# ImIntheMiddle/VATL4Pose-WACV2024

Hardware: AMD Instinct MI355X
Metric: frames/sec pose-infer+uncertainty, 256x192 17-kp (higher is better)
Workload: dtype f32; 1 GPU; SimpleBaseline-R50 256x192 inference + decode + local-peak + THC-L1, 1024-frame synthetic video per GPU; frames_per_gpu=1024, batch=1024, tracks=4, parallelism=frame-sharded x1

## Files before the change

### include/vatl_hip.h

```cpp
#ifndef VATL_HIP_H
#define VATL_HIP_H

#include <stdint.h>

#ifdef __cplusplus
extern "C" {
#endif

#define VATL_VERSION 100
#define VATL_EINVAL  (-1)
#define VATL_ELAUNCH (-2)

int         vatl_version(void);
const char* vatl_last_error(void);

int vatl_flop_meter_begin(void);
int vatl_flop_meter_end(double* direct_flops, double* winograd_flops, int64_t* direct_launches, int64_t* winograd_launches);
#define VATL_ROUTE_NAMES "igemm,igemm_bnbwd,igemm_dma,persistent_1x1,streamk,rows_1x1,bottleneck_chain,stem_pool,halo_3x3," \
                         "winograd,winograd_2h,winograd_bnbwd,winograd_persist,winograd_c32,wgrad,winograd_wgrad,winograd_wgrad_2h," \
                         "winograd_wgrad_table,winograd_f4,winograd_f4_bnbwd,gemm1x1_ring,winograd_deconv43,winograd_s2_43,stem_pool_w1d," \
                         "chain_proj,chain_step"
int vatl_flop_meter_routes(int64_t* counts, int n);


// ... 30 lines not shown
int64_t vatl_winograd_c32_weight_floats(void);
int vatl_pack_winograd_c32_weight(const float* w, float* u, void* stream);
int vatl_conv3x3_winograd_c32_supported(int N, int H, int W, int Cin, int Cout);
int vatl_conv3x3_winograd_c32_fwd(const float* x, const float* u, const float* scale, const float* bias, const float* residual, float* y, int N, int H, int W,
                                  int relu, void* stream);

int64_t vatl_winograd_f4_weight_floats(int Cout, int Cin);
int vatl_pack_winograd_f4_weight(const float* w, float* u, int Cout, int Cin, int data_gradient, void* stream);
int vatl_conv3x3_winograd_f4_supported(int N, int H, int W, int Cin, int Cout);
int vatl_conv3x3_winograd_f4_fwd(const float* x, const float* u, const float* scale, const float* bias, const float* residual, float* y, int N, int H, int W,
                                 int Cin, int Cout, int relu, void* stream);
int64_t vatl_winograd_f4_stats_row_blocks(int64_t N, int H, int W);
int vatl_conv3x3_winograd_f4_fwd_stats(const float* x, const float* u, float* y, double* stats, int64_t* row_blocks_used, int N, int H, int W, int Cin, int Cout,
                                       void* stream);
int vatl_conv3x3_winograd_f4_fwd_bnbwd(const float* x, const float* u, const float* residual, float* y, int N, int H, int W, int Cin, int Cout, const float* bn_z,
                                       const float* bn_mask_y, const float* bn_scale, const float* bn_bias, const float* bn_mean, const float* bn_invstd,
                                       double* stats, int64_t* row_blocks_used, void* stream);

int vatl_conv1x1_rows_supported(int K1, int K2, int N, int64_t M);
int vatl_conv1x1_rows_fwd(const float* a, const float* x2, const float* w, const float* scale, const float* bias, const float* residual, float* y,
                          int64_t M, int K1, int K2, int N, int relu, void* stream);

int vatl_bottleneck_chain_supported(int Cmid, int Cout, int Cnext, int64_t M);
int vatl_bottleneck_chain_fwd(const float* a, const float* w3, const float* scale3, const float* bias3, const float* skip, float* t,
                              const float* w1, const float* scale1, const float* bias1, float* y1, int64_t M, int Cmid, int Cout,
                              int Cnext, void* stream);

int vatl_chain_proj_supported(int Cmid, int Cout, int Cnext, int64_t M);
int vatl_chain_proj_fwd(const float* a, const float* x2, const float* w, const float* scale, const float* bias, float* t, const float* w1,
                        const float* scale1, const float* bias1, float* y1, int64_t M, int Cmid, int Cout, int Cnext, int relu, void* stream);
int vatl_chain_step_supported(int Cmid, int Cout, int Cnext, int64_t M);
int vatl_chain_step_fwd(const float* a, const float* w3, const float* scale3, const float* bias3, const float* skip, float* t, const float* w1,
                        const float* scale1, const float* bias1, float* y1, int64_t M, int Cmid, int Cout, int Cnext, void* stream);

int vatl_tune_set(int knob, int value);
int vatl_set_splitk_workspace(float* workspace, int64_t floats);
int vatl_set_splitk_workspace_thread(float* workspace, int64_t floats);
int64_t vatl_streamk_workspace_bytes(void);
int vatl_set_streamk_workspace_thread(void* workspace, int64_t bytes);
int vatl_conv_cout_pad(int Cout);
int vatl_conv2d_fwd(const float* x, const float* w, const float* scale, const float* bias, const float* residual,
                    float* y, int N, int H, int W, int Cin, int Cout, int CoutPad, int R, int S, int stride, int pad,
                    int relu, int out_nchw, void* stream);

int vatl_deconv4x4s2_fwd(const float* x, const float* w, const float* scale, const float* bias, float* y,
                         int N, int H, int W, int Cin, int Cout, int CoutPad, int relu, void* stream);

int vatl_maxpool3x3s2_fwd(const float* x, float* y, int N, int H, int W, int C, void* stream);
int vatl_gap_fwd(const float* x, float* y, int N, int HW, int C, void* stream);

int vatl_pixelshuffle2_fwd(const float* x, float* y, int N, int H, int W, int C, void* stream);
int vatl_se_scale_add_relu(const float* x, const float* gate, const float* residual, float* y, int N, int HW, int C, void* stream);
int vatl_fuse_upsample_add(const float* base, const float* z0, int shift0, const float* z1, int shift1, const float* z2, int shift2,
                           float* y, int N, int H, int W, int C, int relu, void* stream);
int vatl_upsample_nearest_bwd(const float* dy, const float* yact_or_null, float* dz, int N, int H, int W, int C, int shift, void* stream);
int vatl_gap_bwd(const float* dy, float* dx, int N, int HW, int C, void* stream);


int vatl_decode_argmax_affine(const float* hm, const float* bbox, float* coords, float* maxvals, int32_t* idx,
                              int N, int J, int H, int W, void* stream);
int vatl_decode_pose(const float* hm, const float* bbox, float* kpts, int32_t* idx, float* hp, double* pose_score,
                     int N, int J, int H, int W, void* stream);

int vatl_thc_pairs(const float* a, const float* b, int64_t stride_a, int64_t stride_b, float* out,
                   int P, int J, int HW, int norm, void* stream);
int vatl_thc_combine(const float* pair, const uint8_t* is_prev, const uint8_t* is_next, float* thc, int N, void* stream);
// ... 260 lines not shown
```

### vatl4pose-wacv2024_amd/alphapose/models/hip_engine.py

```python
from __future__ import annotations

import time
import weakref

import torch
import torch.nn as nn

import vatl_hip as vh

MAX_CHUNK = 1024



WINOGRAD = True
ROWS_GEMM = True
ROWS_GEMM_K = (128, 256)
WINO_C32 = True
WINO_F4 = True
DECONV_43 = True
S2_43 = True


class _Conv:
    __slots__ = ("w", "u", "u32", "u4", "us2", "wsrc", "wino", "c32", "f4", "s2", "scale", "bias", "cout", "r", "s", "stride", "pad")
# ... 83 lines not shown
        if WINOGRAD and dc.weight.shape[0] % 16 == 0 and self.cout % 4 == 0:
            self.u = vh.pack_winograd_deconv_weight(dc.weight.detach())
        self.w = vh.pack_deconv_weight(dc.weight.detach())
        self.scale, self.bias = vh.bn_fold(_d(bn.weight), _d(bn.bias), bn.running_mean, bn.running_var, bn.eps)

    def __call__(self, x, relu=True):
        if self.u is not None and not vh.latency_mode():
            if self.d43 and self.u43 is None and vh.deconv4x4s2_winograd43_supported(x.shape[0], x.shape[1], x.shape[2], x.shape[3], self.cout):
                self.u43 = vh.pack_winograd_deconv43_weight(self.wsrc)
            return vh.deconv4x4s2_winograd_fwd(x, self.u, self.scale, self.bias, self.cout, relu, u43=self.u43)
        return vh.deconv4x4s2_fwd(x, self.w, self.scale, self.bias, self.cout, relu)


def _d(p):
    return None if p is None else p.detach()


FUSE_PROJ = True


class _BottleneckPlan:
    def __init__(self, blk):
        self.c1 = _Conv(blk.conv1, blk.bn1)
        self.c2 = _DeformConv(blk) if getattr(blk, "with_dcn", False) else _Conv(blk.conv2, blk.bn2)
        self.c3 = _Conv(blk.conv3, blk.bn3)
        self.proj = _Conv(blk.downsample[0], blk.downsample[1]) if blk.downsample is not None else None
        self.dual = None
        if (FUSE_PROJ and self.proj is not None and type(self) is _BottleneckPlan and self.proj.r == 1 and self.c3.cout >= 128
                and blk.conv3.in_channels % 32 == 0 and blk.downsample[0].in_channels % 32 == 0):
            w, b = vh.pack_conv1x1_dual_weight(blk.conv3.weight.detach(), self.c3.scale, self.c3.bias, blk.downsample[0].weight.detach(),
                                               self.proj.scale, self.proj.bias)
            self.dual = (w, b, self.proj.stride)

    def __call__(self, x, out=None, y1=None, nxt=None):
        y = y1 if y1 is not None else self.c1(x, relu=True)
        y = self.c2(y, relu=True)
        return self.tail(y, x, out=out, nxt=nxt)

    def tail(self, y, x, out=None, nxt=None):
        if self.dual is not None:
            if (ROWS_GEMM and self.dual[2] == 1 and y.shape[-1] == 64 and x.shape[-1] == 64 and not vh.latency_mode()
                    and vh.conv1x1_rows_supported(64, 64, self.c3.cout, y.shape[0] * y.shape[1] * y.shape[2])):
                if nxt is not None and FUSE_CHAIN_PROJ and vh.chain_proj_supported(64, self.c3.cout, nxt[0].shape[0], y.shape[0] * y.shape[1] * y.shape[2]):
                    return vh.conv1x1_rows_fwd(y, self.dual[0], None, self.dual[1], self.c3.cout, True, x2=x, out=out, next_conv1=nxt)
                t = vh.conv1x1_rows_fwd(y, self.dual[0], None, self.dual[1], self.c3.cout, True, x2=x, out=out)
            else:
                t = vh.conv1x1_dual_fwd(y, x, self.dual[0], self.dual[1], self.c3.cout, self.dual[2], True, out=out)
        else:
            skip = x if self.proj is None else self.proj(x, relu=False)
            t = self.c3(y, relu=True, residual=skip, out=out)
        return t if nxt is None else (t, None)


FUSE_CHAIN = True
FUSE_CHAIN_PROJ = True
FUSE_CHAIN_STEP = True


def _conv1_of(nxt, cout):
    if (type(nxt) is _BottleneckPlan and (nxt.c1.r, nxt.c1.stride, nxt.c1.pad) == (1, 1, 0) and nxt.c1.scale is not None and nxt.c1.cout == cout
            and not vh.latency_mode()):
        return nxt.c1.w, nxt.c1.scale, nxt.c1.bias
    return None


def _run_blocks(blocks, x, out=None):
    y1 = None
    for k, b in enumerate(blocks):
        last = k == len(blocks) - 1
        o = out if last else None
        if type(b) is not _BottleneckPlan:
            x, y1 = b(x), None
            continue
        nxt = None if last else blocks[k + 1]
        m = x.shape[0] * x.shape[1] * x.shape[2]
        chain = (FUSE_CHAIN and b.proj is None and not vh.latency_mode() and b.c3.scale is not None
                 and vh.bottleneck_chain_supported(b.c3.w.shape[-1], b.c3.cout, 0, m))
        if not chain:
            c1 = _conv1_of(nxt, 64) if b.dual is not None and FUSE_CHAIN_PROJ else None
            x, y1 = b(x, out=o, y1=y1, nxt=c1) if c1 is not None else (b(x, out=o, y1=y1), None)
            continue
        y = b.c2(y1 if y1 is not None else b.c1(x, relu=True), relu=True)
        link, step = _conv1_of(nxt, 64), _conv1_of(nxt, 128) if FUSE_CHAIN_STEP else None
        if link is not None and vh.bottleneck_chain_supported(b.c3.w.shape[-1], b.c3.cout, 64, m):
            x, y1 = vh.bottleneck_chain_fwd(y, b.c3.w, b.c3.scale, b.c3.bias, x, *link, out=o)
        elif step is not None and vh.chain_step_supported(b.c3.w.shape[-1], b.c3.cout, 128, m):
            x, y1 = vh.bottleneck_chain_fwd(y, b.c3.w, b.c3.scale, b.c3.bias, x, out=o, next_stage_conv1=step)
        else:
            x, y1 = vh.bottleneck_chain_fwd(y, b.c3.w, b.c3.scale, b.c3.bias, x, out=o)[0], None
    return x


FUSE_STEM = True
STEM_W1D = True


def _stem_pool_weight(net):
    c = net.conv1
    ok = (FUSE_STEM and tuple(c.weight.shape) == (64, 3, 7, 7) and c.stride == (2, 2) and c.padding == (3, 3) and c.bias is None
          and isinstance(net.maxpool, nn.MaxPool2d) and net.maxpool.kernel_size in (3, (3, 3)) and net.maxpool.stride in (2, (2, 2))
          and net.maxpool.padding in (1, (1, 1)) and not net.maxpool.ceil_mode)
    return vh.pack_stem_pool_weight(c.weight.detach()) if ok else None


class _TrunkPlan:
    def __init__(self, net):
        self.stem = _Conv(net.conv1, net.bn1)
        self.stem_pw = _stem_pool_weight(net)
        self.stem_src, self.stem_u1d = net.conv1.weight.detach(), None
        self.blocks = [_BottleneckPlan(b) for stage in net.stages() for b in stage]

    def _stem(self, x_nchw):
        if self.stem_pw is not None and not vh.latency_mode() and vh.stem_pool_supported(x_nchw.shape[2], x_nchw.shape[3]):
            u1d = None
            if STEM_W1D and vh.stem_pool_w1d_supported(x_nchw.shape[2], x_nchw.shape[3]):
                if self.stem_u1d is None:
                    self.stem_u1d = vh.pack_stem_pool_w1d_weight(self.stem_src)
                u1d = self.stem_u1d
            return vh.stem_pool_fwd(x_nchw, self.stem_pw, self.stem.scale, self.stem.bias, u1d=u1d)
        x = vh.nchw_to_nhwc(x_nchw, 4)
# ... 398 lines not shown
```

### vatl4pose-wacv2024_amd/csrc/bottleneck_chain.hip

```cpp
#include "common.h"
#include "buffer.h"

namespace vatl {

struct ChainParams {
    const float* a;
    const float* w3;
    const float* scale3;
    const float* bias3;
    const float* res;
    float* t;
    const float* w1;
    const float* scale1;
    const float* bias1;
    float* out2;
    int M, N2, relu3;
    int m_tiles;
    unsigned a_bytes, t_bytes, o_bytes, w3_bytes, w1_bytes;
};

constexpr unsigned BOOB = 0xFFFFFFFFu;

constexpr int BT_LDT = 260;
constexpr int BT_AS = 32 * 64;
// ... 128 lines not shown
#pragma unroll
                    for (int w = 1; w < 4; ++w) {
                        const f32x4 q = *reinterpret_cast<const f32x4*>(&Ts[w * (32 * 68) + row * 68 + q4 * 4]);
#pragma unroll
                        for (int c = 0; c < 4; ++c) sum[c] += q[c];
                    }
                    f32x4 o;
#pragma unroll
                    for (int c = 0; c < 4; ++c) o[c] = fmaxf(sum[c] * s1[c] + b1[c], 0.f);
                    buf_store4(orr, ((unsigned)(mt * 32 + row) * 64u + (unsigned)q4 * 4u) * 4u, o);
                }
            }
        }
        if constexpr (SECOND) asm volatile("s_waitcnt vmcnt(10)" ::: "memory");
        else asm volatile("s_waitcnt vmcnt(8)" ::: "memory");
    }
}


struct FormParams {
    const float* a;
    const float* x2;
    const float* w3;
    const float* scale3;
    const float* bias3;
    const float* res;
    float* t;
    const float* w1;
    const float* scale1;
    const float* bias1;
    float* y;
    int m_tiles, relu3;
    unsigned a_bytes, t_bytes, y_bytes;
};

__device__ __forceinline__ unsigned uadd(unsigned s_part, unsigned v_part) {
#if defined(__HIP_DEVICE_COMPILE__)
    unsigned r;
    asm("v_add_u32 %0, %1, %2" : "=v"(r) : "s"(s_part), "v"(v_part));
    return r;
#else
    return s_part + v_part;
#endif
}

constexpr int CF_TS = 4 * 32 * 64;

template <bool PROJ>
__global__ __launch_bounds__(256, 2) void chain_form_kernel(FormParams p) {
    constexpr int K1 = PROJ ? 128 : 64, G1 = K1 / 8, AS = 32 * K1, N2 = PROJ ? 64 : 128;
    extern __shared__ __attribute__((aligned(16))) float smem[];
    float* As = smem;
    float* Ts = smem + 2 * AS;
    const int tid = threadIdx.x, lane = tid & 63, wave = __builtin_amdgcn_readfirstlane(tid >> 6);
    const int fr = lane & 31, h = lane >> 5;
    const int nblk = gridDim.x;

    const __amdgpu_buffer_rsrc_t ar = buf_rsrc(p.a, p.a_bytes);
    const __amdgpu_buffer_rsrc_t xr = buf_rsrc(PROJ ? p.x2 : p.a, PROJ ? p.a_bytes : 0u);
    const __amdgpu_buffer_rsrc_t w3r = buf_rsrc(p.w3, 256u * K1 * 4u);
    const __amdgpu_buffer_rsrc_t w1r = buf_rsrc(p.w1, (unsigned)N2 * 256u * 4u);
    const __amdgpu_buffer_rsrc_t tr = buf_rsrc(p.t, p.t_bytes);
    const __amdgpu_buffer_rsrc_t rr = buf_rsrc(p.res ? p.res : p.t, p.res ? p.t_bytes : 0u);
    const __amdgpu_buffer_rsrc_t yr = buf_rsrc(p.y, p.y_bytes);

    f32x4 w3f[2][G1];
#pragma unroll
    for (int nb = 0; nb < 2; ++nb)
#pragma unroll
        for (int g = 0; g < G1; ++g) w3f[nb][g] = buf_load4(w3r, (unsigned)(((wave * 64 + nb * 32 + fr) * K1 + 8 * g + 4 * h) * 4));
    float sc3[2], bi3[2];
#pragma unroll
    for (int nb = 0; nb < 2; ++nb) {
        const int n = wave * 64 + nb * 32 + fr;
        sc3[nb] = p.scale3 ? p.scale3[n] : 1.f;
        bi3[nb] = p.bias3 ? p.bias3[n] : 0.f;
    }
    const int l16 = lane & 15, j = lane >> 4;
    const int n1 = PROJ ? wave * 16 + l16 : wave * 32 + fr;
    f32x4 w1f[PROJ ? 16 : 32];
#pragma unroll
    for (int g = 0; g < (PROJ ? 16 : 32); ++g) w1f[g] = buf_load4(w1r, (unsigned)((n1 * 256 + (PROJ ? 16 * g + 4 * j : 8 * g + 4 * h)) * 4));
    const float sc1 = p.scale1 ? p.scale1[n1] : 1.f, bi1 = p.bias1 ? p.bias1[n1] : 0.f;
    const float lo3 = p.relu3 ? 0.f : -INFINITY;

    const int c4 = lane, r0 = wave;
    int ax[4], tq[4], tw[2], tx[PROJ ? 2 : 4];
#pragma unroll
    for (int k = 0; k < 4; ++k) {
        ax[k] = fr * K1 + (((2 * k + h) ^ (fr & 7)) << 2);
        tq[k] = 2 * AS + 4 * h * 64 + ((((fr >> 2) ^ (4 * h) ^ k) << 2) | (fr & 3));
    }
#pragma unroll
    for (int k = 0; k < 2; ++k) tw[k] = 2 * AS + (c4 >> 4) * 2048 + (((c4 & 15) ^ (r0 | 4 * k)) << 2);
#pragma unroll
// ... 27 lines not shown
            __builtin_amdgcn_raw_ptr_buffer_load_lds(rr, (lds_void*)(Ts + wave * 2048 + u * 256), 16,
                                                     uadd((unsigned)mt * (32u * 1024u) + (unsigned)u * 4096u + (unsigned)wave * 256u, vs[u & 1]), 0, 0, 0);
    };

    int mt = blockIdx.x, buf = 0;
    a_dma(0, mt);
    asm volatile("s_waitcnt vmcnt(0)" ::: "memory");
    for (; mt < p.m_tiles; mt += nblk, buf ^= 1) {
        lds_barrier();
        if constexpr (!PROJ) skip_dma(mt);
        a_dma(buf ^ 1, mt + nblk);
        __builtin_amdgcn_sched_barrier(0);
        const int abase = buf * AS, tqbase = wave * 2048;
#pragma unroll
        for (int nb = 0; nb < 2; ++nb) {
            f32x16 acc;
#pragma unroll
            for (int e = 0; e < 16; ++e) acc[e] = 0.f;
#pragma unroll
            for (int g = 0; g < G1; ++g) {
                const f32x4 af = *reinterpret_cast<const f32x4*>(smem + abase + ax[g & 3] + 32 * (g >> 2));
#pragma unroll
                for (int tt = 0; tt < 4; ++tt) acc = __builtin_amdgcn_mfma_f32_32x32x2f32(af[tt], w3f[nb][g][tt], acc, 0, 0, 0);
            }
            if (!PROJ && nb == 0) asm volatile("s_waitcnt vmcnt(2)" ::: "memory");
#pragma unroll
            for (int e = 0; e < 16; ++e) {
                float* q = smem + tqbase + tq[e & 3] + 64 * ((e & 3) + 8 * (e >> 2)) + 32 * nb;
                const float v = acc[e] * sc3[nb] + bi3[nb];
                *q = fmaxf(v + (PROJ ? 0.f : *q), lo3);
            }
        }
        lds_barrier();
#pragma unroll
        for (int u = 0; u < 8; ++u)
            buf_store4(tr, uadd((unsigned)mt * (32u * 1024u) + (unsigned)(r0 + 4 * u) * 1024u, (unsigned)c4 * 16u),
                       *reinterpret_cast<const f32x4*>(smem + r0 * 64 + tw[u & 1] + 256 * u));
        const unsigned ytile = (unsigned)mt * (32u * N2 * 4u) + (unsigned)wave * (PROJ ? 64u : 128u);
        if constexpr (PROJ) {
            f32x4 acc2[2] = {f32x4{0.f, 0.f, 0.f, 0.f}, f32x4{0.f, 0.f, 0.f, 0.f}};
#pragma unroll
            for (int q = 0; q < 16; ++q) {
                f32x4 tf[2];
#pragma unroll
                for (int rb = 0; rb < 2; ++rb) tf[rb] = *reinterpret_cast<const f32x4*>(smem + tx[q & 1] + 32 * ((q >> 1) & 1) + 2048 * (q >> 2) + 1024 * rb);
#pragma unroll
                for (int tt = 0; tt < 4; ++tt)
#pragma unroll
                    for (int rb = 0; rb < 2; ++rb) acc2[rb] = __builtin_amdgcn_mfma_f32_16x16x4f32(tf[rb][tt], w1f[q][tt], acc2[rb], 0, 0, 0);
            }
#pragma unroll
            for (int rb = 0; rb < 2; ++rb)
#pragma unroll
                for (int r = 0; r < 4; ++r) buf_store1(yr, uadd(ytile + (unsigned)(rb * 16 + r) * (N2 * 4u), vy), fmaxf(acc2[rb][r] * sc1 + bi1, 0.f));
            asm volatile("s_waitcnt vmcnt(16)" ::: "memory");
        } else {
            f32x16 acc2;
#pragma unroll
            for (int e = 0; e < 16; ++e) acc2[e] = 0.f;
#pragma unroll
            for (int g = 0; g < 32; ++g) {
                const f32x4 tf = *reinterpret_cast<const f32x4*>(smem + tx[g & 3] + 32 * ((g >> 2) & 1) + 2048 * (g >> 3));
#pragma unroll
                for (int tt = 0; tt < 4; ++tt) acc2 = __builtin_amdgcn_mfma_f32_32x32x2f32(tf[tt], w1f[g][tt], acc2, 0, 0, 0);
            }
#pragma unroll
            for (int e = 0; e < 16; ++e) buf_store1(yr, uadd(ytile + (unsigned)((e & 3) + 8 * (e >> 2)) * (N2 * 4u), vy), fmaxf(acc2[e] * sc1 + bi1 + 0.f, 0.f));
            asm volatile("s_waitcnt vmcnt(24)" ::: "memory");
        }
    }
}

}

using namespace vatl;

static bool chain_shape_ok(int Cmid, int Cout, int Cnext, int64_t M) {
    return Cmid == 64 && Cout == 256 && (Cnext == 64 || Cnext == 0) && M > 0 && (M + 32) * 256 < (1LL << 30);
}

extern "C" int vatl_bottleneck_chain_supported(int Cmid, int Cout, int Cnext, int64_t M) { return chain_shape_ok(Cmid, Cout, Cnext, M) ? 1 : 0; }

extern "C" int vatl_bottleneck_chain_fwd(const float* a, const float* w3, const float* scale3, const float* bias3, const float* skip, float* t, const float* w1,
                                         const float* scale1, const float* bias1, float* y1, int64_t M, int Cmid, int Cout, int Cnext, void* stream) {
    if (!a || !w3 || !t || (Cnext != 0) != (w1 != nullptr) || (w1 && !y1)) return fail(VATL_EINVAL, "bottleneck_chain_fwd: bad arguments");
    if (!chain_shape_ok(Cmid, Cout, Cnext, M)) return fail(VATL_EINVAL, "bottleneck_chain_fwd: serves 64 -> 256 (-> 64) channels and (M + 32) * 256 < 2^30 pixels x channels");
    ChainParams p{};
    p.a = a; p.w3 = w3; p.scale3 = scale3; p.bias3 = bias3; p.res = skip; p.t = t; p.w1 = w1; p.scale1 = scale1; p.bias1 = bias1; p.out2 = y1;
    p.M = (int)M; p.N2 = 64; p.relu3 = 1; p.m_tiles = (int)((M + 31) / 32);
    p.a_bytes = (unsigned)(M * 64 * 4); p.t_bytes = (unsigned)(M * 256 * 4); p.o_bytes = (unsigned)(M * 64 * 4); p.w3_bytes = 256 * 64 * 4; p.w1_bytes = 64 * 256 * 4;
    const int smem = BT_FLOATS * (int)sizeof(float);
    static std::atomic<unsigned> c0{0}, c1{0};
    const double padded = (double)p.m_tiles * 32.0;
    if (w1) {
        auto kern = bottleneck_chain_kernel<true>;
        if (int rc = ensure_dynamic_lds(reinterpret_cast<const void*>(kern), smem, c1, "bottleneck_chain")) return rc;
        const int grid = p.m_tiles < 512 ? p.m_tiles : 512;
        hipLaunchKernelGGL(kern, dim3(grid), dim3(256), smem, (hipStream_t)stream, p);
        meter_add(0, 2.0 * padded * 256.0 * 64.0 * 2.0);
        meter_route(kRouteChain);
    } else {
        auto kern = bottleneck_chain_kernel<false>;
        if (int rc = ensure_dynamic_lds(reinterpret_cast<const void*>(kern), smem, c0, "bottleneck_chain")) return rc;
        const int grid = p.m_tiles < 512 ? p.m_tiles : 512;
        hipLaunchKernelGGL(kern, dim3(grid), dim3(256), smem, (hipStream_t)stream, p);
        meter_add(0, 2.0 * padded * 256.0 * 64.0);
        meter_route(kRouteChain);
    }
    return check_launch("bottleneck_chain");
}

static bool form_shape_ok(int Cmid, int Cout, int Cnext, int want_next, int64_t M) {
    return Cmid == 64 && Cout == 256 && Cnext == want_next && M > 0 && (M + 32) * 256 < (1LL << 30);
}

extern "C" int vatl_chain_proj_supported(int Cmid, int Cout, int Cnext, int64_t M) { return form_shape_ok(Cmid, Cout, Cnext, 64, M) ? 1 : 0; }
extern "C" int vatl_chain_step_supported(int Cmid, int Cout, int Cnext, int64_t M) { return form_shape_ok(Cmid, Cout, Cnext, 128, M) ? 1 : 0; }

static int chain_form_launch(bool proj, FormParams p, int64_t M, void* stream) {
    const int N2 = proj ? 64 : 128, K1 = proj ? 128 : 64;
    const char* what = proj ? "chain_proj" : "chain_step";
    p.m_tiles = (int)((M + 31) / 32);
    p.a_bytes = (unsigned)(M * 64 * 4); p.t_bytes = (unsigned)(M * 256 * 4); p.y_bytes = (unsigned)(M * N2 * 4);
    const int smem = (2 * 32 * K1 + CF_TS) * (int)sizeof(float);
    static std::atomic<unsigned> c[2] = {{0}, {0}};
    void (*kern)(FormParams) = chain_form_kernel<false>;
    if (proj) kern = chain_form_kernel<true>;
    if (int rc = ensure_dynamic_lds(reinterpret_cast<const void*>(kern), smem, c[proj], what)) return rc;
    const int grid = p.m_tiles < 512 ? p.m_tiles : 512;
    hipLaunchKernelGGL(kern, dim3(grid), dim3(256), smem, (hipStream_t)stream, p);
    meter_add(0, 2.0 * ((double)p.m_tiles * 32.0) * 256.0 * (double)(K1 + N2));
    meter_route(proj ? kRouteChainProj : kRouteChainStep);
    return check_launch(what);
}

extern "C" int vatl_chain_proj_fwd(const float* a, const float* x2, const float* w, const float* scale, const float* bias, float* t, const float* w1, const float* scale1,
                                   const float* bias1, float* y1, int64_t M, int Cmid, int Cout, int Cnext, int relu, void* stream) {
    if (!a || !x2 || !w || !t || !w1 || !y1) return fail(VATL_EINVAL, "chain_proj_fwd: bad arguments");
    if (!form_shape_ok(Cmid, Cout, Cnext, 64, M)) return fail(VATL_EINVAL, "chain_proj_fwd: serves 64 + 64 -> 256 -> 64 channels and (M + 32) * 256 < 2^30 pixels x channels");
    FormParams p{};
    p.a = a; p.x2 = x2; p.w3 = w; p.scale3 = scale; p.bias3 = bias; p.t = t; p.w1 = w1; p.scale1 = scale1; p.bias1 = bias1; p.y = y1; p.relu3 = relu;
    return chain_form_launch(true, p, M, stream);
}

extern "C" int vatl_chain_step_fwd(const float* a, const float* w3, const float* scale3, const float* bias3, const float* skip, float* t, const float* w1,
                                   const float* scale1, const float* bias1, float* y1, int64_t M, int Cmid, int Cout, int Cnext, void* stream) {
    if (!a || !w3 || !t || !w1 || !y1) return fail(VATL_EINVAL, "chain_step_fwd: bad arguments");
    if (!form_shape_ok(Cmid, Cout, Cnext, 128, M)) return fail(VATL_EINVAL, "chain_step_fwd: serves 64 -> 256 -> 128 channels and (M + 32) * 256 < 2^30 pixels x channels");
    FormParams p{};
    p.a = a; p.w3 = w3; p.scale3 = scale3; p.bias3 = bias3; p.res = skip; p.t = t; p.w1 = w1; p.scale1 = scale1; p.bias1 = bias1; p.y = y1; p.relu3 = 1;
    return chain_form_launch(false, p, M, stream);
}
```

### vatl4pose-wacv2024_amd/vatl_hip/__init__.py

```python
from __future__ import annotations

import ctypes as C
import os
import threading as _threading

import torch

_HERE = os.path.dirname(os.path.abspath(__file__))
LIB_PATH = os.environ.get("VATL_HIP_LIB") or os.path.join(_HERE, "libvatl_hip.so")

_p = C.c_void_p
_i = C.c_int
_f = C.c_float
_d = C.c_double
_i64 = C.c_int64

SIGNATURES = {
    "vatl_version": (_i, []),
    "vatl_last_error": (C.c_char_p, []),
    "vatl_flop_meter_begin": (_i, []),
    "vatl_flop_meter_end": (_i, [_p, _p, _p, _p]),
    "vatl_flop_meter_routes": (_i, [_p, _i]),
    "vatl_nchw_to_nhwc": (_i, [_p, _p, _i, _i, _i, _i, _i, _p]),
    "vatl_nhwc_to_nchw": (_i, [_p, _p, _i, _i, _i, _i, _p]),
    "vatl_pack_conv_weight": (_i, [_p, _p, _i, _i, _i, _i, _i, _i, _i, _p]),
    "vatl_pack_deconv4x4s2_weight": (_i, [_p, _p, _i, _i, _i, _p]),
    "vatl_pack_conv1x1_dual_weight": (_i, [_p, _p, _p, _p, _p, _p, _p, _p, _i, _i, _i, _i, _p]),
    "vatl_conv1x1_dual_fwd": (_i, [_p, _p, _p, _p, _p, _i, _i, _i, _i, _i, _i, _i, _i, _i, _i, _i, _p]),
    "vatl_winograd_c32_weight_floats": (_i64, []),
    "vatl_pack_winograd_c32_weight": (_i, [_p, _p, _p]),
    "vatl_conv3x3_winograd_c32_supported": (_i, [_i, _i, _i, _i, _i]),
    "vatl_conv3x3_winograd_c32_fwd": (_i, [_p, _p, _p, _p, _p, _p, _i, _i, _i, _i, _p]),
    "vatl_winograd_f4_weight_floats": (_i64, [_i, _i]),
    "vatl_pack_winograd_f4_weight": (_i, [_p, _p, _i, _i, _i, _p]),
    "vatl_winograd_f4_stats_row_blocks": (_i64, [_i64, _i, _i]),
    "vatl_conv3x3_winograd_f4_fwd_stats": (_i, [_p, _p, _p, _p, _p, _i, _i, _i, _i, _i, _p]),
    "vatl_conv3x3_winograd_f4_fwd_bnbwd": (_i, [_p, _p, _p, _p, _i, _i, _i, _i, _i, _p, _p, _p, _p, _p, _p, _p, _p, _p]),
    "vatl_conv3x3_winograd_f4_supported": (_i, [_i, _i, _i, _i, _i]),
    "vatl_conv3x3_winograd_f4_fwd": (_i, [_p, _p, _p, _p, _p, _p, _i, _i, _i, _i, _i, _i, _p]),
    "vatl_conv1x1_rows_supported": (_i, [_i, _i, _i, _i64]),
    "vatl_conv1x1_rows_fwd": (_i, [_p, _p, _p, _p, _p, _p, _p, _i64, _i, _i, _i, _i, _p]),
    "vatl_bottleneck_chain_supported": (_i, [_i, _i, _i, _i64]),
    "vatl_bottleneck_chain_fwd": (_i, [_p, _p, _p, _p, _p, _p, _p, _p, _p, _p, _i64, _i, _i, _i, _p]),
    "vatl_chain_proj_supported": (_i, [_i, _i, _i, _i64]),
    "vatl_chain_proj_fwd": (_i, [_p, _p, _p, _p, _p, _p, _p, _p, _p, _p, _i64, _i, _i, _i, _i, _p]),
    "vatl_chain_step_supported": (_i, [_i, _i, _i, _i64]),
    "vatl_chain_step_fwd": (_i, [_p, _p, _p, _p, _p, _p, _p, _p, _p, _p, _i64, _i, _i, _i, _p]),
    "vatl_stem_pool_weight_floats": (_i64, []),
    "vatl_pack_stem_pool_weight": (_i, [_p, _p, _p]),
    "vatl_stem_pool_supported": (_i, [_i, _i]),
    "vatl_stem_pool_w1d_weight_floats": (_i64, []),
    "vatl_pack_stem_pool_w1d_weight": (_i, [_p, _p, _p]),
    "vatl_stem_pool_w1d_supported": (_i, [_i, _i]),
    "vatl_stem7x7s2_pool_w1d_fwd": (_i, [_p] * 5 + [_i] * 3 + [_p]),
    "vatl_stem7x7s2_pool_fwd": (_i, [_p, _p, _p, _p, _p, _i, _i, _i, _p]),
    "vatl_stem3_weight_floats": (_i64, []),
    "vatl_pack_stem3_weight": (_i, [_p, _p, _p]),
    "vatl_stem3x3s2_fwd": (_i, [_p, _p, _p, _p, _p, _i, _i, _i, _p]),
    "vatl_bn_fold": (_i, [_p, _p, _p, _p, _p, _f, _p, _p, _i, _p]),
    "vatl_tune_set": (_i, [_i, _i]),
    "vatl_set_splitk_workspace": (_i, [_p, _i64]),
    "vatl_set_splitk_workspace_thread": (_i, [_p, _i64]),
    "vatl_streamk_workspace_bytes": (_i64, []),
    "vatl_set_streamk_workspace_thread": (_i, [_p, _i64]),
    "vatl_conv_cout_pad": (_i, [_i]),
    "vatl_conv2d_fwd": (_i, [_p, _p, _p, _p, _p, _p, _i, _i, _i, _i, _i, _i, _i, _i, _i, _i, _i, _i, _p]),
    "vatl_deconv4x4s2_fwd": (_i, [_p, _p, _p, _p, _p, _i, _i, _i, _i, _i, _i, _i, _p]),
    "vatl_maxpool3x3s2_fwd": (_i, [_p, _p, _i, _i, _i, _i, _p]),
    "vatl_gap_fwd": (_i, [_p, _p, _i, _i, _i, _p]),
    "vatl_pixelshuffle2_fwd": (_i, [_p, _p, _i, _i, _i, _i, _p]),
    "vatl_se_scale_add_relu": (_i, [_p, _p, _p, _p, _i, _i, _i, _p]),
    "vatl_fuse_upsample_add": (_i, [_p, _p, _i, _p, _i, _p, _i, _p, _i, _i, _i, _i, _i, _p]),
    "vatl_upsample_nearest_bwd": (_i, [_p, _p, _p, _i, _i, _i, _i, _i, _p]),
    "vatl_gap_bwd": (_i, [_p, _p, _i, _i, _i, _p]),
    "vatl_decode_argmax_affine": (_i, [_p, _p, _p, _p, _p, _i, _i, _i, _i, _p]),
    "vatl_decode_pose": (_i, [_p, _p, _p, _p, _p, _p, _i, _i, _i, _i, _p]),
    "vatl_thc_pairs": (_i, [_p, _p, _i64, _i64, _p, _i, _i, _i, _i, _p]),
    "vatl_thc_combine": (_i, [_p, _p, _p, _p, _i, _p]),
    "vatl_localpeak_mean": (_i, [_p, _p, _p, _p, _i, _i, _i, _i, _f, _p]),
    "vatl_hybrid_ae_wpu": (_i, [_p, _p, _p, _i, _i, _i, _p, _p, _i, _p]),
# ... 592 lines not shown
    n, h, w_, k1 = a.shape
    k2 = 0 if x2 is None else x2.shape[-1]
    assert w.numel() >= cout * (k1 + k2) and (x2 is None or tuple(x2.shape[:3]) == (n, h, w_)) and (residual is None or tuple(residual.shape) == (n, h, w_, cout))
    y = out if out is not None else torch.empty((n, h, w_, cout), device=a.device, dtype=torch.float32)
    assert a.is_contiguous() and y.is_contiguous() and (x2 is None or x2.is_contiguous()) and (residual is None or residual.is_contiguous())
    if next_conv1 is not None:
        w1, scale1, bias1 = next_conv1
        cnext = w1.shape[0]
        if x2 is None or k2 != k1 or residual is not None:
            raise VatlError("conv1x1_rows_fwd: next_conv1 goes with the two-source form (a, x2 of 64 channels each) and no residual")
        assert w1.numel() == cnext * cout
        y1 = y1_out if y1_out is not None else torch.empty((n, h, w_, cnext), device=a.device, dtype=torch.float32)
        assert y1.is_contiguous()
        _check(lib().vatl_chain_proj_fwd(_ptr(a), _ptr(x2), _ptr(w), _ptr(scale), _ptr(bias), _ptr(y), _ptr(w1), _ptr(scale1), _ptr(bias1), _ptr(y1),
                                         n * h * w_, k1, cout, cnext, int(relu), _stream()), "vatl_chain_proj_fwd")
        return y, y1
    _check(lib().vatl_conv1x1_rows_fwd(_ptr(a), _ptr(x2), _ptr(w), _ptr(scale), _ptr(bias), _ptr(residual), _ptr(y), n * h * w_, k1, k2, cout, int(relu),
                                       _stream()), "vatl_conv1x1_rows_fwd")
    return y


def bottleneck_chain_supported(cmid: int, cout: int, cnext: int, m: int) -> bool:
    return bool(lib().vatl_bottleneck_chain_supported(cmid, cout, cnext, m))


def chain_proj_supported(cmid: int, cout: int, cnext: int, m: int) -> bool:
    return bool(lib().vatl_chain_proj_supported(cmid, cout, cnext, m))


def chain_step_supported(cmid: int, cout: int, cnext: int, m: int) -> bool:
    return bool(lib().vatl_chain_step_supported(cmid, cout, cnext, m))


def bottleneck_chain_fwd(a, w3, scale3, bias3, skip, w1=None, scale1=None, bias1=None, out=None, y1_out=None, next_stage_conv1=None):
    n, h, w_, cmid = a.shape
    cout = w3.shape[0]
    step = next_stage_conv1 is not None
    if step:
        if w1 is not None:
            raise VatlError("bottleneck_chain_fwd: w1 and next_stage_conv1 are exclusive")
        w1, scale1, bias1 = next_stage_conv1
    cnext = 0 if w1 is None else w1.shape[0]
    assert w3.numel() == cout * cmid and (w1 is None or w1.numel() == cnext * cout) and (skip is None or tuple(skip.shape) == (n, h, w_, cout))
    t = out if out is not None else torch.empty((n, h, w_, cout), device=a.device, dtype=torch.float32)
    assert t.is_contiguous() and a.is_contiguous() and (skip is None or skip.is_contiguous())
    y1 = None if w1 is None else (y1_out if y1_out is not None else torch.empty((n, h, w_, cnext), device=a.device, dtype=torch.float32))
    assert y1 is None or y1.is_contiguous()
    fn, name = (lib().vatl_chain_step_fwd, "vatl_chain_step_fwd") if step else (lib().vatl_bottleneck_chain_fwd, "vatl_bottleneck_chain_fwd")
    _check(fn(_ptr(a), _ptr(w3), _ptr(scale3), _ptr(bias3), _ptr(skip), _ptr(t), _ptr(w1), _ptr(scale1), _ptr(bias1), _ptr(y1),
              n * h * w_, cmid, cout, cnext, _stream()), name)
    return t, y1


def stem3_fwd(x_nchw: torch.Tensor, w_packed: torch.Tensor, scale: torch.Tensor, bias: torch.Tensor, out=None) -> torch.Tensor:
    n, c, h, w = x_nchw.shape
    if c != 3:
        raise VatlError(f"stem3_fwd: expected 3 input channels, got {c}")
    y = out if out is not None else torch.empty((n, h // 2, w // 2, 64), device=x_nchw.device, dtype=torch.float32)
    _check(lib().vatl_stem3x3s2_fwd(_ptr(x_nchw), _ptr(w_packed), _ptr(scale), _ptr(bias), _ptr(y), n, h, w, _stream()), "vatl_stem3x3s2_fwd")
    return y


def stem_pool_supported(h: int, w: int) -> bool:
    return bool(lib().vatl_stem_pool_supported(int(h), int(w)))


def stem_pool_w1d_supported(h: int, w: int) -> bool:
    return bool(lib().vatl_stem_pool_w1d_supported(int(h), int(w)))


def stem_pool_w1d_fwd(x_nchw: torch.Tensor, u1d: torch.Tensor, scale: torch.Tensor, bias: torch.Tensor, out=None) -> torch.Tensor:
    n, c, h, w = x_nchw.shape
    if c != 3:
        raise VatlError(f"stem_pool_w1d_fwd: expected 3 input channels, got {c}")
    y = out if out is not None else torch.empty((n, h // 4, w // 4, 64), device=x_nchw.device, dtype=torch.float32)
    _check(lib().vatl_stem7x7s2_pool_w1d_fwd(_ptr(x_nchw), _ptr(u1d), _ptr(scale), _ptr(bias), _ptr(y), n, h, w, _stream()), "vatl_stem7x7s2_pool_w1d_fwd")
    return y


def stem_pool_fwd(x_nchw: torch.Tensor, w_packed: torch.Tensor, scale: torch.Tensor, bias: torch.Tensor, out=None, u1d=None) -> torch.Tensor:
# ... 1218 lines not shown
```

Before: 17630 frames/s.

## Write only stride-2 decimated skip output from chain-step kernel into compact tensor

At the stage transition, the last layer1-style block's output feeds only the next block's conv1 (already fused in the kernel) and its stride-2 projection shortcut. The kernel therefore now stores only even-row, even-column pixels of the 256-channel output into a compact (N, H/2, W/2, 256) tensor. Odd pixels are routed to an out-of-range buffer offset and dropped. The next block then runs its dual conv3+projection with stride 1 on the compact input. This cuts roughly three quarters of the full-resolution activation write and the later strided read, at the cost of per-pixel index math and a new kernel variant.

```diff
diff --git a/include/vatl_hip.h b/include/vatl_hip.h
--- a/include/vatl_hip.h
+++ b/include/vatl_hip.h
@@ -86,6 +86,9 @@
 int vatl_chain_step_supported(int Cmid, int Cout, int Cnext, int64_t M);
 int vatl_chain_step_fwd(const float* a, const float* w3, const float* scale3, const float* bias3, const float* skip, float* t, const float* w1,
                         const float* scale1, const float* bias1, float* y1, int64_t M, int Cmid, int Cout, int Cnext, void* stream);
+int vatl_chain_step_s2_fwd(const float* a, const float* w3, const float* scale3, const float* bias3, const float* skip, float* tc, int64_t tc_floats,
+                           const float* w1, const float* scale1, const float* bias1, float* y1, int64_t M, int H, int W, int Cmid, int Cout, int Cnext,
+                           void* stream);
 
 int vatl_tune_set(int knob, int value);
 int vatl_set_splitk_workspace(float* workspace, int64_t floats);
diff --git a/vatl4pose-wacv2024_amd/alphapose/models/hip_engine.py b/vatl4pose-wacv2024_amd/alphapose/models/hip_engine.py
--- a/vatl4pose-wacv2024_amd/alphapose/models/hip_engine.py
+++ b/vatl4pose-wacv2024_amd/alphapose/models/hip_engine.py
@@ -139,12 +139,16 @@
                                                self.proj.scale, self.proj.bias)
             self.dual = (w, b, self.proj.stride)
 
-    def __call__(self, x, out=None, y1=None, nxt=None):
+    def __call__(self, x, out=None, y1=None, nxt=None, x_decimated=False):
         y = y1 if y1 is not None else self.c1(x, relu=True)
         y = self.c2(y, relu=True)
-        return self.tail(y, x, out=out, nxt=nxt)
-
-    def tail(self, y, x, out=None, nxt=None):
+        return self.tail(y, x, out=out, nxt=nxt, x_decimated=x_decimated)
+
+    def tail(self, y, x, out=None, nxt=None, x_decimated=False):
+        if x_decimated:
+            assert self.dual is not None and x.shape[:3] == y.shape[:3]
+            t = vh.conv1x1_dual_fwd(y, x, self.dual[0], self.dual[1], self.c3.cout, 1, True, out=out)
+            return t if nxt is None else (t, None)
         if self.dual is not None:
             if (ROWS_GEMM and self.dual[2] == 1 and y.shape[-1] == 64 and x.shape[-1] == 64 and not vh.latency_mode()
                     and vh.conv1x1_rows_supported(64, 64, self.c3.cout, y.shape[0] * y.shape[1] * y.shape[2])):
@@ -162,6 +166,7 @@
 FUSE_CHAIN = True
 FUSE_CHAIN_PROJ = True
 FUSE_CHAIN_STEP = True
+CHAIN_STEP_COMPACT = True
 
 
 def _conv1_of(nxt, cout):
@@ -172,7 +177,7 @@
 
 
 def _run_blocks(blocks, x, out=None):
-    y1 = None
+    y1, decimated = None, False
     for k, b in enumerate(blocks):
         last = k == len(blocks) - 1
         o = out if last else None
@@ -184,15 +189,17 @@
         chain = (FUSE_CHAIN and b.proj is None and not vh.latency_mode() and b.c3.scale is not None
                  and vh.bottleneck_chain_supported(b.c3.w.shape[-1], b.c3.cout, 0, m))
         if not chain:
-            c1 = _conv1_of(nxt, 64) if b.dual is not None and FUSE_CHAIN_PROJ else None
-            x, y1 = b(x, out=o, y1=y1, nxt=c1) if c1 is not None else (b(x, out=o, y1=y1), None)
+            c1 = _conv1_of(nxt, 64) if b.dual is not None and FUSE_CHAIN_PROJ and not decimated else None
+            x, y1 = b(x, out=o, y1=y1, nxt=c1) if c1 is not None else (b(x, out=o, y1=y1, x_decimated=decimated), None)
+            decimated = False
             continue
         y = b.c2(y1 if y1 is not None else b.c1(x, relu=True), relu=True)
         link, step = _conv1_of(nxt, 64), _conv1_of(nxt, 128) if FUSE_CHAIN_STEP else None
         if link is not None and vh.bottleneck_chain_supported(b.c3.w.shape[-1], b.c3.cout, 64, m):
             x, y1 = vh.bottleneck_chain_fwd(y, b.c3.w, b.c3.scale, b.c3.bias, x, *link, out=o)
         elif step is not None and vh.chain_step_supported(b.c3.w.shape[-1], b.c3.cout, 128, m):
-            x, y1 = vh.bottleneck_chain_fwd(y, b.c3.w, b.c3.scale, b.c3.bias, x, out=o, next_stage_conv1=step)
+            decimated = CHAIN_STEP_COMPACT and o is None and nxt.dual is not None and nxt.dual[2] == 2
+            x, y1 = vh.bottleneck_chain_fwd(y, b.c3.w, b.c3.scale, b.c3.bias, x, out=o, next_stage_conv1=step, skip_out_stride2=decimated)
         else:
             x, y1 = vh.bottleneck_chain_fwd(y, b.c3.w, b.c3.scale, b.c3.bias, x, out=o)[0], None
     return x
diff --git a/vatl4pose-wacv2024_amd/csrc/bottleneck_chain.hip b/vatl4pose-wacv2024_amd/csrc/bottleneck_chain.hip
--- a/vatl4pose-wacv2024_amd/csrc/bottleneck_chain.hip
+++ b/vatl4pose-wacv2024_amd/csrc/bottleneck_chain.hip
@@ -184,7 +184,12 @@
     float* y;
     int m_tiles, relu3;
     unsigned a_bytes, t_bytes, y_bytes;
+    unsigned ts_bytes;
+    int H, W, Hc, Wc;
+    FastDivU d_hw, d_w;
 };
+
+constexpr unsigned CF_DROP = 0xFFFFF000u;
 
 __device__ __forceinline__ unsigned uadd(unsigned s_part, unsigned v_part) {
 #if defined(__HIP_DEVICE_COMPILE__)
@@ -198,8 +203,9 @@
 
 constexpr int CF_TS = 4 * 32 * 64;
 
-template <bool PROJ>
+template <bool PROJ, bool COMPACT = false>
 __global__ __launch_bounds__(256, 2) void chain_form_kernel(FormParams p) {
+    static_assert(!(PROJ && COMPACT), "the compact T output belongs to form S");
     constexpr int K1 = PROJ ? 128 : 64, G1 = K1 / 8, AS = 32 * K1, N2 = PROJ ? 64 : 128;
     extern __shared__ __attribute__((aligned(16))) float smem[];
     float* As = smem;
@@ -212,7 +218,7 @@
     const __amdgpu_buffer_rsrc_t xr = buf_rsrc(PROJ ? p.x2 : p.a, PROJ ? p.a_bytes : 0u);
     const __amdgpu_buffer_rsrc_t w3r = buf_rsrc(p.w3, 256u * K1 * 4u);
     const __amdgpu_buffer_rsrc_t w1r = buf_rsrc(p.w1, (unsigned)N2 * 256u * 4u);
-    const __amdgpu_buffer_rsrc_t tr = buf_rsrc(p.t, p.t_bytes);
+    const __amdgpu_buffer_rsrc_t tr = buf_rsrc(p.t, p.ts_bytes);
     const __amdgpu_buffer_rsrc_t rr = buf_rsrc(p.res ? p.res : p.t, p.res ? p.t_bytes : 0u);
     const __amdgpu_buffer_rsrc_t yr = buf_rsrc(p.y, p.y_bytes);
 
@@ -306,10 +312,17 @@
             }
         }
         lds_barrier();
-#pragma unroll
-        for (int u = 0; u < 8; ++u)
-            buf_store4(tr, uadd((unsigned)mt * (32u * 1024u) + (unsigned)(r0 + 4 * u) * 1024u, (unsigned)c4 * 16u),
-                       *reinterpret_cast<const f32x4*>(smem + r0 * 64 + tw[u & 1] + 256 * u));
+        if constexpr (!COMPACT) {
+#pragma unroll
+            for (int u = 0; u < 8; ++u)
+                buf_store4(tr, uadd((unsigned)mt * (32u * 1024u) + (unsigned)(r0 + 4 * u) * 1024u, (unsigned)c4 * 16u),
+                           *reinterpret_cast<const f32x4*>(smem + r0 * 64 + tw[u & 1] + 256 * u));
+        }
+        auto tc_off = [&](int u) {
+            const int pix = mt * 32 + r0 + 4 * u, img = fdiv(pix, p.d_hw), rem = pix - img * (p.H * p.W), y = fdiv(rem, p.d_w), x = rem - y * p.W;
+            const unsigned odd = 0u - (unsigned)((y | x) & 1);
+            return uadd((CF_DROP & odd) | ((unsigned)((img * p.Hc + (y >> 1)) * p.Wc + (x >> 1)) * 1024u & ~odd), (unsigned)c4 * 16u);
+        };
         const unsigned ytile = (unsigned)mt * (32u * N2 * 4u) + (unsigned)wave * (PROJ ? 64u : 128u);
         if constexpr (PROJ) {
             f32x4 acc2[2] = {f32x4{0.f, 0.f, 0.f, 0.f}, f32x4{0.f, 0.f, 0.f, 0.f}};
@@ -332,11 +345,18 @@
             f32x16 acc2;
 #pragma unroll
             for (int e = 0; e < 16; ++e) acc2[e] = 0.f;
+            if constexpr (COMPACT) __builtin_amdgcn_sched_barrier(0);
 #pragma unroll
             for (int g = 0; g < 32; ++g) {
                 const f32x4 tf = *reinterpret_cast<const f32x4*>(smem + tx[g & 3] + 32 * ((g >> 2) & 1) + 2048 * (g >> 3));
+                f32x4 trow;
+                if (COMPACT && g < 8) trow = *reinterpret_cast<const f32x4*>(smem + r0 * 64 + tw[g & 1] + 256 * g);
 #pragma unroll
                 for (int tt = 0; tt < 4; ++tt) acc2 = __builtin_amdgcn_mfma_f32_32x32x2f32(tf[tt], w1f[g][tt], acc2, 0, 0, 0);
+                if (COMPACT && g < 8) {
+                    buf_store4(tr, tc_off(g), trow);
+                    __builtin_amdgcn_sched_barrier(0);
+                }
             }
 #pragma unroll
             for (int e = 0; e < 16; ++e) buf_store1(yr, uadd(ytile + (unsigned)((e & 3) + 8 * (e >> 2)) * (N2 * 4u), vy), fmaxf(acc2[e] * sc1 + bi1 + 0.f, 0.f));
@@ -396,11 +416,19 @@
     const char* what = proj ? "chain_proj" : "chain_step";
     p.m_tiles = (int)((M + 31) / 32);
     p.a_bytes = (unsigned)(M * 64 * 4); p.t_bytes = (unsigned)(M * 256 * 4); p.y_bytes = (unsigned)(M * N2 * 4);
+    if (p.W) {
+        p.Hc = (p.H + 1) / 2; p.Wc = (p.W + 1) / 2;
+        p.ts_bytes = (unsigned)(M / ((int64_t)p.H * p.W) * p.Hc * p.Wc * 256 * 4);
+        p.d_hw = make_fastdiv((unsigned)(p.H * p.W)); p.d_w = make_fastdiv((unsigned)p.W);
+    } else {
+        p.ts_bytes = p.t_bytes;
+    }
     const int smem = (2 * 32 * K1 + CF_TS) * (int)sizeof(float);
-    static std::atomic<unsigned> c[2] = {{0}, {0}};
+    static std::atomic<unsigned> c[3] = {{0}, {0}, {0}};
     void (*kern)(FormParams) = chain_form_kernel<false>;
     if (proj) kern = chain_form_kernel<true>;
-    if (int rc = ensure_dynamic_lds(reinterpret_cast<const void*>(kern), smem, c[proj], what)) return rc;
+    if (p.W) kern = chain_form_kernel<false, true>;
+    if (int rc = ensure_dynamic_lds(reinterpret_cast<const void*>(kern), smem, c[p.W ? 2 : proj], what)) return rc;
     const int grid = p.m_tiles < 512 ? p.m_tiles : 512;
     hipLaunchKernelGGL(kern, dim3(grid), dim3(256), smem, (hipStream_t)stream, p);
     meter_add(0, 2.0 * ((double)p.m_tiles * 32.0) * 256.0 * (double)(K1 + N2));
@@ -425,3 +453,17 @@
     p.a = a; p.w3 = w3; p.scale3 = scale3; p.bias3 = bias3; p.res = skip; p.t = t; p.w1 = w1; p.scale1 = scale1; p.bias1 = bias1; p.y = y1; p.relu3 = 1;
     return chain_form_launch(false, p, M, stream);
 }
+
+extern "C" int vatl_chain_step_s2_fwd(const float* a, const float* w3, const float* scale3, const float* bias3, const float* skip, float* tc, int64_t tc_floats,
+                                      const float* w1, const float* scale1, const float* bias1, float* y1, int64_t M, int H, int W, int Cmid, int Cout, int Cnext,
+                                      void* stream) {
+    if (!a || !w3 || !tc || !w1 || !y1) return fail(VATL_EINVAL, "chain_step_s2_fwd: bad arguments");
+    if (!form_shape_ok(Cmid, Cout, Cnext, 128, M)) return fail(VATL_EINVAL, "chain_step_s2_fwd: serves 64 -> 256 -> 128 channels and (M + 32) * 256 < 2^30 pixels x channels");
+    if (H < 1 || W < 1 || (int64_t)H * W > M || M % ((int64_t)H * W)) return fail(VATL_EINVAL, "chain_step_s2_fwd: %lld pixels are not whole %d x %d images", (long long)M, H, W);
+    const int64_t want = M / ((int64_t)H * W) * ((H + 1) / 2) * ((W + 1) / 2) * 256;
+    if (tc_floats != want) return fail(VATL_EINVAL, "chain_step_s2_fwd: the compact tensor has %lld values, (N, ceil(H / 2), ceil(W / 2), 256) has %lld", (long long)tc_floats, (long long)want);
+    FormParams p{};
+    p.a = a; p.w3 = w3; p.scale3 = scale3; p.bias3 = bias3; p.res = skip; p.t = tc; p.w1 = w1; p.scale1 = scale1; p.bias1 = bias1; p.y = y1; p.relu3 = 1;
+    p.H = H; p.W = W;
+    return chain_form_launch(false, p, M, stream);
+}
diff --git a/vatl4pose-wacv2024_amd/vatl_hip/__init__.py b/vatl4pose-wacv2024_amd/vatl_hip/__init__.py
--- a/vatl4pose-wacv2024_amd/vatl_hip/__init__.py
+++ b/vatl4pose-wacv2024_amd/vatl_hip/__init__.py
@@ -46,6 +46,7 @@
     "vatl_chain_proj_fwd": (_i, [_p, _p, _p, _p, _p, _p, _p, _p, _p, _p, _i64, _i, _i, _i, _i, _p]),
     "vatl_chain_step_supported": (_i, [_i, _i, _i, _i64]),
     "vatl_chain_step_fwd": (_i, [_p, _p, _p, _p, _p, _p, _p, _p, _p, _p, _i64, _i, _i, _i, _p]),
+    "vatl_chain_step_s2_fwd": (_i, [_p, _p, _p, _p, _p, _p, _i64, _p, _p, _p, _p, _i64, _i, _i, _i, _i, _i, _p]),
     "vatl_stem_pool_weight_floats": (_i64, []),
     "vatl_pack_stem_pool_weight": (_i, [_p, _p, _p]),
     "vatl_stem_pool_supported": (_i, [_i, _i]),
@@ -704,7 +705,7 @@
     return bool(lib().vatl_chain_step_supported(cmid, cout, cnext, m))
 
 
-def bottleneck_chain_fwd(a, w3, scale3, bias3, skip, w1=None, scale1=None, bias1=None, out=None, y1_out=None, next_stage_conv1=None):
+def bottleneck_chain_fwd(a, w3, scale3, bias3, skip, w1=None, scale1=None, bias1=None, out=None, y1_out=None, next_stage_conv1=None, skip_out_stride2=False):
     n, h, w_, cmid = a.shape
     cout = w3.shape[0]
     step = next_stage_conv1 is not None
@@ -712,12 +713,21 @@
         if w1 is not None:
             raise VatlError("bottleneck_chain_fwd: w1 and next_stage_conv1 are exclusive")
         w1, scale1, bias1 = next_stage_conv1
+    elif skip_out_stride2:
+        raise VatlError("bottleneck_chain_fwd: skip_out_stride2 goes with next_stage_conv1")
     cnext = 0 if w1 is None else w1.shape[0]
     assert w3.numel() == cout * cmid and (w1 is None or w1.numel() == cnext * cout) and (skip is None or tuple(skip.shape) == (n, h, w_, cout))
-    t = out if out is not None else torch.empty((n, h, w_, cout), device=a.device, dtype=torch.float32)
+    t_shape = (n, (h + 1) // 2, (w_ + 1) // 2, cout) if skip_out_stride2 else (n, h, w_, cout)
+    if skip_out_stride2 and out is not None and tuple(out.shape) != t_shape:
+        raise VatlError(f"bottleneck_chain_fwd: out is {tuple(out.shape)}, the launch writes {t_shape}")
+    t = out if out is not None else torch.empty(t_shape, device=a.device, dtype=torch.float32)
     assert t.is_contiguous() and a.is_contiguous() and (skip is None or skip.is_contiguous())
     y1 = None if w1 is None else (y1_out if y1_out is not None else torch.empty((n, h, w_, cnext), device=a.device, dtype=torch.float32))
     assert y1 is None or y1.is_contiguous()
+    if skip_out_stride2:
+        _check(lib().vatl_chain_step_s2_fwd(_ptr(a), _ptr(w3), _ptr(scale3), _ptr(bias3), _ptr(skip), _ptr(t), t.numel(), _ptr(w1), _ptr(scale1), _ptr(bias1),
+                                            _ptr(y1), n * h * w_, h, w_, cmid, cout, cnext, _stream()), "vatl_chain_step_s2_fwd")
+        return t, y1
     fn, name = (lib().vatl_chain_step_fwd, "vatl_chain_step_fwd") if step else (lib().vatl_bottleneck_chain_fwd, "vatl_bottleneck_chain_fwd")
     _check(fn(_ptr(a), _ptr(w3), _ptr(scale3), _ptr(bias3), _ptr(skip), _ptr(t), _ptr(w1), _ptr(scale1), _ptr(bias1), _ptr(y1),
               n * h * w_, cmid, cout, cnext, _stream()), name)
```

Result: no change. 17730 frames/s, median of 6 (+0.6%).
